# 0xMiden/miden-vm

Measured on AMD Instinct MI355X. Metric: trace rows/sec proved (2^20-row trace, 96-bit sec), higher is better.
Workload: dtype u64 (Goldilocks field, p = 2^64 - 2^32 + 1); 1 GPU; full proof of miden:20:51:8 (DummyMidenAir 2^20 x 51 + 8 EF aux), 96-bit production PCS params (blowup 8, FRI arity 4, 27 queries, PoW 4/12/16), Poseidon2 LMCS; trace resident in HBM, transcript on host; log_trace_rows=20, main_width=51, aux_width_ef=8, log_blowup=3, proof_bytes=137697, parallelism=1 GPU

## Files before the change

### miden-vm_amd/csrc/deep.hip

```cpp
#include "gl.cuh"
#include "kernels.hpp"

__global__ __launch_bounds__(256) void k_bary_weights(const u64* tw, int log_n, u64 g, e2 y0, e2 y1, u64* w0, u64* w1) {
  const size_t n = (size_t)1 << log_n;
  const size_t base = (size_t)blockIdx.x * 1024 + threadIdx.x;
  const size_t half = n >> 1;
  u64 xs[4], nrm[8], pre[8];
  e2 den[8];
#pragma unroll
  for (int k = 0; k < 4; k++) {
    size_t r = base + (size_t)k * 256;
    u64 x = 0;
    if (r < n) x = gl_mul(g, half ? (r < half ? tw[r] : gl_neg(tw[r - half])) : 1);
    xs[k] = x;
    den[2 * k] = e2_sub(y0, e2_make(x));
    den[2 * k + 1] = e2_sub(y1, e2_make(x));
  }
  u64 run = 1;
#pragma unroll
  for (int k = 0; k < 8; k++) {
    nrm[k] = gl_sub(gl_sqr(den[k].c0), gl_mul7(gl_sqr(den[k].c1)));
    pre[k] = run;
    run = gl_mul(run, nrm[k]);
  }
  u64 inv = gl_inv(run);
#pragma unroll
  for (int k = 7; k >= 0; k--) {
    u64 ni = gl_mul(inv, pre[k]);
    inv = gl_mul(inv, nrm[k]);
    size_t r = base + (size_t)(k >> 1) * 256;
    if (r < n) {
      u64 s = gl_mul(ni, xs[k >> 1]);
      u64* w = (k & 1) ? w1 : w0;
      w[2 * r] = gl_mul(den[k].c0, s);
      w[2 * r + 1] = gl_mul(gl_neg(den[k].c1), s);
    }
  }
}

static constexpr int OOD_ROWS_PER_BLOCK = 8192;
__global__ __launch_bounds__(256) void k_ood_partial(const u64* lde, int log_n, int log_blowup, const u64* w0, const u64* w1,
                                                     u64* partial, unsigned chunks) {
  __shared__ u64 red[4][256];
  const size_t n = (size_t)1 << log_n;
  const size_t col = blockIdx.y, chunk = blockIdx.x;
  const u64* f = lde + ((col << log_blowup) << log_n);
  const size_t r0 = chunk * OOD_ROWS_PER_BLOCK;
  const size_t r1 = r0 + OOD_ROWS_PER_BLOCK < n ? r0 + OOD_ROWS_PER_BLOCK : n;
  e2 a0 = e2_make(0), a1 = e2_make(0);
  for (size_t r = r0 + threadIdx.x; r < r1; r += 256) {
    u64 v = f[r];
    a0 = e2_add(a0, e2_mulf(e2{w0[2 * r], w0[2 * r + 1]}, v));
    a1 = e2_add(a1, e2_mulf(e2{w1[2 * r], w1[2 * r + 1]}, v));
  }
  red[0][threadIdx.x] = a0.c0; red[1][threadIdx.x] = a0.c1; red[2][threadIdx.x] = a1.c0; red[3][threadIdx.x] = a1.c1;
  __syncthreads();
  for (int s = 128; s > 0; s >>= 1) {
    if ((int)threadIdx.x < s) {
#pragma unroll
      for (int k = 0; k < 4; k++) red[k][threadIdx.x] = gl_add(red[k][threadIdx.x], red[k][threadIdx.x + s]);
    }
    __syncthreads();
  }
  if (threadIdx.x < 4) partial[(col * chunks + chunk) * 4 + threadIdx.x] = red[threadIdx.x][0];
}

void deep_ood_eval_batch(mh_ctx* c, std::vector<OodJob>& jobs, int log_blowup) {
  struct Weights {
    int log_n;
    size_t coset0;
    e2 y0, y1;
    DevBuf w0, w1;
  };
  std::vector<std::unique_ptr<Weights>> weights;
  struct Slot {
    size_t off = 0, ncol = 0;
    unsigned chunks = 0;
  };
  std::vector<Slot> slots(jobs.size());
  size_t total = 0;
  for (size_t k = 0; k < jobs.size(); k++) {
    OodJob& j = jobs[k];
    const LdeMatrix& m = *j.m;
    if (j.col_end > m.width) j.col_end = m.width;
    j.out0.assign(m.width, e2_make(0));
    j.out1.assign(m.width, e2_make(0));
    if (j.col_begin >= j.col_end) continue;
    const size_t n = (size_t)1 << m.log_n;
    slots[k].ncol = j.col_end - j.col_begin;
    slots[k].chunks = (unsigned)((n + OOD_ROWS_PER_BLOCK - 1) / OOD_ROWS_PER_BLOCK);
    slots[k].off = total;
    total += slots[k].ncol * slots[k].chunks * 4;
  }
  if (!total) return;
  DevBuf partial(total * 8), one;
  for (size_t k = 0; k < jobs.size(); k++) {
    if (!slots[k].ncol) continue;
    const OodJob& j = jobs[k];
    const LdeMatrix& m = *j.m;
    const int log_n = m.log_n;
    const size_t n = (size_t)1 << log_n;
    const u64 g = gl_mul(gl_lde_shift(log_n + log_blowup), gl_pow(gl_two_adic_generator(log_n + log_blowup), m.coset0));
    const u64* tw = log_n ? c->twiddles(log_n, false) : nullptr;
    if (!tw) {
      if (!one.p) {
        one.alloc(8);
        u64 v = 1;
        c->h2d(one.p, &v, 8);
      }
      tw = one.u();
    }
    ProfScope ps(c, "deep_ood_eval", (double)n * 8.0 * slots[k].ncol + 64.0 * n);
    Weights* w = nullptr;
    for (auto& cand : weights)
      if (cand->log_n == log_n && cand->coset0 == m.coset0 && e2_eq(cand->y0, j.y0) && e2_eq(cand->y1, j.y1)) w = cand.get();
    if (!w) {
      weights.emplace_back(new Weights{log_n, m.coset0, j.y0, j.y1, DevBuf(n * 16), DevBuf(n * 16)});
      w = weights.back().get();
      MH_LAUNCH(k_bary_weights, dim3((unsigned)((n + 1023) / 1024)), dim3(256), 0, c->stream, tw, log_n, g, j.y0, j.y1, w->w0.u(), w->w1.u());
    }
    MH_LAUNCH(k_ood_partial, dim3(slots[k].chunks, (unsigned)slots[k].ncol), dim3(256), 0, c->stream,
              m.lde.u() + ((j.col_begin << m.log_cosets) << log_n), log_n, m.log_cosets, w->w0.u(), w->w1.u(), partial.u() + slots[k].off,
              slots[k].chunks);
  }
  std::vector<u64> host(total);
  c->d2h(host.data(), partial.p, total * 8);
  for (size_t k = 0; k < jobs.size(); k++) {
    if (!slots[k].ncol) continue;
    OodJob& j = jobs[k];
    const LdeMatrix& m = *j.m;
    const int log_n = m.log_n;
    const size_t n = (size_t)1 << log_n;
    const u64 g = gl_mul(gl_lde_shift(log_n + log_blowup), gl_pow(gl_two_adic_generator(log_n + log_blowup), m.coset0));
    const u64 g_inv = gl_inv(g), n_inv = gl_inv((u64)n % GL_P);
    const e2 s0 = e2_mulf(e2_sub(e2_exp_pow2(e2_mulf(j.y0, g_inv), log_n), e2_make(1)), n_inv);
    const e2 s1 = e2_mulf(e2_sub(e2_exp_pow2(e2_mulf(j.y1, g_inv), log_n), e2_make(1)), n_inv);
    for (size_t col = 0; col < slots[k].ncol; col++) {
      e2 a0 = e2_make(0), a1 = e2_make(0);
      for (unsigned ch = 0; ch < slots[k].chunks; ch++) {
        const u64* p = host.data() + slots[k].off + (col * slots[k].chunks + ch) * 4;
        a0 = e2_add(a0, e2{p[0], p[1]});
        a1 = e2_add(a1, e2{p[2], p[3]});
      }
      j.out0[j.col_begin + col] = e2_mul(a0, s0);
      j.out1[j.col_begin + col] = e2_mul(a1, s1);
    }
  }
}
void deep_ood_eval_matrix(mh_ctx* c, const LdeMatrix& m, int log_blowup, e2 y0, e2 y1, std::vector<e2>& out0, std::vector<e2>& out1,
                          size_t col_begin, size_t col_end) {
  std::vector<OodJob> jobs(1);
  jobs[0].m = &m; jobs[0].y0 = y0; jobs[0].y1 = y1; jobs[0].col_begin = col_begin; jobs[0].col_end = col_end;
  deep_ood_eval_batch(c, jobs, log_blowup);
  out0.swap(jobs[0].out0);
  out1.swap(jobs[0].out1);
}

static constexpr int DEEP_MAX_MATS = 128;
static constexpr unsigned DEEP_FLUSH = 128;
#ifndef DEEP_UNROLL
#define DEEP_UNROLL 2
#endif
#ifndef DEEP_PTS_N
#define DEEP_PTS_N 1
#endif
static constexpr int DEEP_PTS = DEEP_PTS_N;
struct DeepMat {
  const u64* lde;
  u32 width, coef_off;
  int log_n;
};
struct DeepArgs {
  DeepMat m[DEEP_MAX_MATS];
  int n_mats, log_n, log_blowup;
  const u64* negc;
  const u64* tw;
  const u64* coset_x;
  e2 z0, z1, fred0, fred1, beta;
  u64* out;
};

template <bool PLANES>
__global__ __launch_bounds__(256) void k_deep_assemble(DeepArgs a) {
  const size_t N = (size_t)1 << a.log_n;
  const size_t j = blockIdx.y;
  const size_t base = (size_t)blockIdx.x * (256 * DEEP_PTS) + threadIdx.x;
  size_t r[DEEP_PTS];
#pragma unroll
  for (int k = 0; k < DEEP_PTS; k++) r[k] = base + (size_t)k * 256;
  e2 neg[DEEP_PTS];
  u64 w[DEEP_PTS][2][6];
#pragma unroll
  for (int k = 0; k < DEEP_PTS; k++) {
    neg[k] = e2_make(0);
#pragma unroll
    for (int e = 0; e < 2; e++)
#pragma unroll
      for (int i = 0; i < 6; i++) w[k][e][i] = 0;
  }
  auto flush = [&]() {
    const u64 C[6] = {1ULL, 1ULL << 22, 1ULL << 44, 1ULL << 32, 1ULL << 54, GL_EPS << 12};
#pragma unroll
    for (int k = 0; k < DEEP_PTS; k++) {
      u64 s0 = w[k][0][0], s1 = w[k][1][0];
#pragma unroll
      for (int i = 1; i < 6; i++) {
        s0 = gl_add(s0, gl_mul(w[k][0][i], C[i]));
        s1 = gl_add(s1, gl_mul(w[k][1][i], C[i]));
      }
      neg[k] = e2_add(neg[k], e2{s0, s1});
#pragma unroll
      for (int e = 0; e < 2; e++)
#pragma unroll
        for (int i = 0; i < 6; i++) w[k][e][i] = 0;
    }
  };
  u32 pending = 0;
#pragma unroll 1
  for (int mi = 0; mi < a.n_mats; mi++) {
    const DeepMat m = a.m[mi];
    const size_t nm_mask = ((size_t)1 << m.log_n) - 1;
    const u64* colp = m.lde + (j << m.log_n);
    const size_t cstride = (size_t)1 << (m.log_n + a.log_blowup);
#pragma unroll DEEP_UNROLL
    for (u32 cidx = 0; cidx < m.width; cidx++) {
      const u64 cf0 = a.negc[2 * (m.coef_off + cidx)], cf1 = a.negc[2 * (m.coef_off + cidx) + 1];
      u32 al[2][3];
#pragma unroll
      for (int i = 0; i < 3; i++) {
        al[0][i] = (u32)(cf0 >> (22 * i)) & 0x3FFFFFu;
        al[1][i] = (u32)(cf1 >> (22 * i)) & 0x3FFFFFu;
      }
#pragma unroll
      for (int k = 0; k < DEEP_PTS; k++) {
        if (r[k] < N) {
          const u64 v = colp[r[k] & nm_mask];
          const u32 v0 = (u32)v, v1 = (u32)(v >> 32);
#pragma unroll
          for (int e = 0; e < 2; e++) {
            w[k][e][0] += (u64)al[e][0] * v0;
            w[k][e][1] += (u64)al[e][1] * v0;
            w[k][e][2] += (u64)al[e][2] * v0;
            w[k][e][3] += (u64)al[e][0] * v1;
            w[k][e][4] += (u64)al[e][1] * v1;
            w[k][e][5] += (u64)al[e][2] * v1;
          }
        }
      }
      colp += cstride;
      if (++pending == DEEP_FLUSH) {
        flush();
        pending = 0;
      }
    }
  }
  flush();
  const size_t half = N >> 1;
  const u64 cx = a.coset_x[j];
  e2 den[2 * DEEP_PTS];
  u64 nrm[2 * DEEP_PTS], pre[2 * DEEP_PTS];
#pragma unroll
  for (int k = 0; k < DEEP_PTS; k++) {
    u64 x = 0;
    if (r[k] < N) x = gl_mul(cx, half ? (r[k] < half ? a.tw[r[k]] : gl_neg(a.tw[r[k] - half])) : 1);
    den[2 * k] = e2_sub(a.z0, e2_make(x));
    den[2 * k + 1] = e2_sub(a.z1, e2_make(x));
  }
  u64 run = 1;
#pragma unroll
  for (int k = 0; k < 2 * DEEP_PTS; k++) {
    nrm[k] = gl_sub(gl_sqr(den[k].c0), gl_mul7(gl_sqr(den[k].c1)));
    pre[k] = run;
    run = gl_mul(run, nrm[k]);
  }
  u64 inv = gl_inv(run);
  e2 qinv[2 * DEEP_PTS];
#pragma unroll
  for (int k = 2 * DEEP_PTS - 1; k >= 0; k--) {
    u64 ni = gl_mul(inv, pre[k]);
    inv = gl_mul(inv, nrm[k]);
    qinv[k] = e2{gl_mul(den[k].c0, ni), gl_mul(gl_neg(den[k].c1), ni)};
  }
#pragma unroll
  for (int k = 0; k < DEEP_PTS; k++) {
    if (r[k] < N) {
      e2 v = e2_mul(qinv[2 * k], e2_add(a.fred0, neg[k]));
      v = e2_add(v, e2_mul(e2_mul(a.beta, qinv[2 * k + 1]), e2_add(a.fred1, neg[k])));
      if constexpr (PLANES) {
        a.out[r[k]] = v.c0;
        a.out[N + r[k]] = v.c1;
      } else {
        ulonglong2* o = reinterpret_cast<ulonglong2*>(a.out + 2 * ((j << a.log_n) + r[k]));
        *o = make_ulonglong2(v.c0, v.c1);
      }
    }
  }
}

__global__ __launch_bounds__(256) void k_deep_interleave(const u64* __restrict__ planes, size_t n, u64* __restrict__ out) {
  const size_t i = (size_t)blockIdx.x * 256 + threadIdx.x;
  if (i >= n) return;
  *reinterpret_cast<ulonglong2*>(out + 2 * i) = make_ulonglong2(planes[i], planes[n + i]);
}

void deep_assemble(mh_ctx* c, const std::vector<const LdeMatrix*>& mats, const std::vector<u32>& coef_off, int log_n, int log_blowup,
                   const std::vector<e2>& negc, e2 z0, e2 z1, e2 fred0, e2 fred1, e2 beta, u64* out, bool one_coset) {
  MH_REQUIRE(mats.size() <= (size_t)DEEP_MAX_MATS, "too many committed matrices for one DEEP pass");
  const int lbl = mats[0]->log_cosets;
  const size_t coset0 = mats[0]->coset0;
  for (auto* m : mats) MH_REQUIRE(m->log_cosets == lbl && m->coset0 == coset0, "internal: matrices cover different cosets");
  const size_t N = (size_t)1 << log_n, B = (size_t)1 << lbl;
  const int L = log_n + log_blowup;
  std::vector<u64> blob;
  for (e2 v : negc) { blob.push_back(v.c0); blob.push_back(v.c1); }
  const size_t o_cx = blob.size();
  const u64 g = gl_lde_shift(L), wK = gl_two_adic_generator(L);
  u64 x = gl_mul(g, gl_pow(wK, coset0));
  for (size_t j = 0; j < B; j++) {
    blob.push_back(x);
    x = gl_mul(x, wK);
  }
  DevBuf dblob(blob.size() * 8), one;
  c->h2d(dblob.p, blob.data(), blob.size() * 8);
  const u64* tw = log_n ? c->twiddles(log_n, false) : nullptr;
  if (!tw) {
    one.alloc(8);
    u64 v = 1;
    c->h2d(one.p, &v, 8);
    tw = one.u();
  }
  MH_REQUIRE(!one_coset || (lbl >= 1 && log_n >= DEEP_ONE_COSET_MIN_LOG_N), "internal: one-coset DEEP assemble needs two cosets to extend to");
  const size_t Ba = one_coset ? 1 : B;
  DeepArgs a{};
  double bytes = 16.0 * N * Ba;
  for (size_t i = 0; i < mats.size(); i++) {
    a.m[i] = DeepMat{mats[i]->lde.u(), (u32)mats[i]->width, coef_off[i], mats[i]->log_n};
    bytes += 8.0 * (double)mats[i]->width * (double)(((size_t)1 << mats[i]->log_n) * Ba);
  }
  a.n_mats = (int)mats.size();
  a.log_n = log_n; a.log_blowup = lbl;
  a.negc = dblob.u(); a.tw = tw; a.coset_x = dblob.u() + o_cx;
  a.z0 = z0; a.z1 = z1; a.fred0 = fred0; a.fred1 = fred1; a.beta = beta; a.out = out;
  const dim3 grid((unsigned)((N + 256 * DEEP_PTS - 1) / (256 * DEEP_PTS)), (unsigned)Ba);
  if (!one_coset) {
    ProfScope ps(c, "deep_assemble", bytes);
    MH_LAUNCH(k_deep_assemble<false>, grid, dim3(256), 0, c->stream, a);
    HIP_CHECK(hipStreamSynchronize(c->stream));
    return;
  }
  DevBuf planes(2 * N * 8), scratch(2 * N * 8), ext(2 * B * N * 8);
  a.out = planes.u();
  {
    ProfScope ps(c, "deep_assemble", bytes);
    MH_LAUNCH(k_deep_assemble<true>, grid, dim3(256), 0, c->stream, a);
  }
  {
    ProfScope ps(c, "deep_extend", 16.0 * N + 3.0 * 16.0 * N * B);
    const std::vector<u64> shifts(blob.begin() + o_cx, blob.begin() + o_cx + B);
    lde_columns(c, planes.u(), 2, log_n, shifts[0], shifts, ext.u(), scratch.u());
    MH_LAUNCH(k_deep_interleave, dim3((unsigned)((B * N + 255) / 256)), dim3(256), 0, c->stream, ext.u(), B * N, out);
  }
  HIP_CHECK(hipStreamSynchronize(c->stream));
}
```

Baseline: 24.98 million trace rows/s.

## Group OOD columns per block and use lazy limb-split accumulation

Adds a grouped out-of-domain evaluation kernel in which each block handles several columns at once, so each barycentric weight load is reused across the group. It also drops per-row Goldilocks reductions: each weight is split into 22-bit limbs and multiplied against 32-bit halves of the value, and the products are accumulated in plain 64-bit sums that are reduced only once at the end. A static assertion bounds the accumulators so no mid-loop flush is needed. The grouped path is on by default and can be turned off with an environment variable. The cost is more registers per thread and a tighter occupancy hint.

```diff
diff --git a/miden-vm_amd/csrc/deep.hip b/miden-vm_amd/csrc/deep.hip
--- a/miden-vm_amd/csrc/deep.hip
+++ b/miden-vm_amd/csrc/deep.hip
@@ -63,6 +63,83 @@
     __syncthreads();
   }
   if (threadIdx.x < 4) partial[(col * chunks + chunk) * 4 + threadIdx.x] = red[threadIdx.x][0];
+}
+
+#ifndef OOD_GROUP_N
+#define OOD_GROUP_N 4
+#endif
+static constexpr int OOD_GROUP = OOD_GROUP_N;
+static constexpr int OOD_ROWS_PER_LANE = OOD_ROWS_PER_BLOCK / 256;
+static_assert(OOD_ROWS_PER_BLOCK % 256 == 0 && (u64)OOD_ROWS_PER_LANE * 2 * 0x3FFFFFULL * 0xFFFFFFFFULL < (1ULL << 60),
+              "k_ood_partial_grouped: an accumulator must stay canonical without a flush");
+__device__ __forceinline__ u64 ood_shift32(u64 w) {
+  const u32 a = (u32)w, b = (u32)(w >> 32);
+  const u32 t = a + b, c = t < a;
+  const u32 sub = b + c;
+  return ((u64)(t + c - (sub != 0)) << 32) | (u32)(0u - sub);
+}
+template <int G>
+__global__ __launch_bounds__(256) __attribute__((amdgpu_waves_per_eu(4))) void k_ood_partial_grouped(
+    const u64* lde, int log_n, int log_blowup, const u64* w0, const u64* w1, u64* partial, unsigned chunks, unsigned ncol) {
+  __shared__ u64 red[4][256];
+  const size_t n = (size_t)1 << log_n;
+  const size_t chunk = blockIdx.x;
+  const unsigned col0 = blockIdx.y * G;
+  const u64* f[G];
+#pragma unroll
+  for (int g = 0; g < G; g++) {
+    const size_t col = col0 + g < ncol ? col0 + g : ncol - 1;
+    f[g] = lde + ((col << log_blowup) << log_n);
+  }
+  const size_t r0 = chunk * OOD_ROWS_PER_BLOCK;
+  const size_t r1 = r0 + OOD_ROWS_PER_BLOCK < n ? r0 + OOD_ROWS_PER_BLOCK : n;
+  u64 acc[G][4][3];
+#pragma unroll
+  for (int g = 0; g < G; g++)
+#pragma unroll
+    for (int k = 0; k < 4; k++)
+#pragma unroll
+      for (int i = 0; i < 3; i++) acc[g][k][i] = 0;
+  for (size_t r = r0 + threadIdx.x; r < r1; r += 256) {
+    const ulonglong2 wa = *reinterpret_cast<const ulonglong2*>(w0 + 2 * r), wb = *reinterpret_cast<const ulonglong2*>(w1 + 2 * r);
+    u32 v0[G], v1[G];
+#pragma unroll
+    for (int g = 0; g < G; g++) {
+      const u64 v = f[g][r];
+      v0[g] = (u32)v;
+      v1[g] = (u32)(v >> 32);
+    }
+    const u64 wk[4] = {wa.x, wa.y, wb.x, wb.y};
+#pragma unroll
+    for (int k = 0; k < 4; k++) {
+      const u64 ws = ood_shift32(wk[k]);
+#pragma unroll
+      for (int i = 0; i < 3; i++) {
+        const u32 l = (u32)(wk[k] >> (22 * i)) & 0x3FFFFFu, ls = (u32)(ws >> (22 * i)) & 0x3FFFFFu;
+#pragma unroll
+        for (int g = 0; g < G; g++) {
+          acc[g][k][i] += (u64)l * v0[g];
+          acc[g][k][i] += (u64)ls * v1[g];
+        }
+      }
+    }
+  }
+#pragma unroll
+  for (int g = 0; g < G; g++) {
+    if (g) __syncthreads();
+#pragma unroll
+    for (int k = 0; k < 4; k++)
+      red[k][threadIdx.x] = gl_add(gl_add(acc[g][k][0], gl_mul(acc[g][k][1], 1ULL << 22)), gl_mul(acc[g][k][2], 1ULL << 44));
+    __syncthreads();
+    for (int s = 128; s > 0; s >>= 1) {
+      if ((int)threadIdx.x < s) {
+#pragma unroll
+        for (int k = 0; k < 4; k++) red[k][threadIdx.x] = gl_add(red[k][threadIdx.x], red[k][threadIdx.x + s]);
+      }
+      __syncthreads();
+    }
+    if (threadIdx.x < 4 && col0 + g < ncol) partial[((size_t)(col0 + g) * chunks + chunk) * 4 + threadIdx.x] = red[threadIdx.x][0];
+  }
 }
 
 void deep_ood_eval_batch(mh_ctx* c, std::vector<OodJob>& jobs, int log_blowup) {
@@ -94,6 +171,11 @@
   }
   if (!total) return;
   DevBuf partial(total * 8), one;
+  const char* grouped_env = getenv("MH_OOD_GROUPED");
+  const bool grouped = !(grouped_env && grouped_env[0] && !atoi(grouped_env));
+  if (grouped) {
+    ProfScope mark(c, "ood_grouped");
+  }
   for (size_t k = 0; k < jobs.size(); k++) {
     if (!slots[k].ncol) continue;
     const OodJob& j = jobs[k];
@@ -119,9 +201,14 @@
       w = weights.back().get();
       MH_LAUNCH(k_bary_weights, dim3((unsigned)((n + 1023) / 1024)), dim3(256), 0, c->stream, tw, log_n, g, j.y0, j.y1, w->w0.u(), w->w1.u());
     }
-    MH_LAUNCH(k_ood_partial, dim3(slots[k].chunks, (unsigned)slots[k].ncol), dim3(256), 0, c->stream,
-              m.lde.u() + ((j.col_begin << m.log_cosets) << log_n), log_n, m.log_cosets, w->w0.u(), w->w1.u(), partial.u() + slots[k].off,
-              slots[k].chunks);
+    const u64* lde0 = m.lde.u() + ((j.col_begin << m.log_cosets) << log_n);
+    if (grouped)
+      MH_LAUNCH(k_ood_partial_grouped<OOD_GROUP>, dim3(slots[k].chunks, (unsigned)((slots[k].ncol + OOD_GROUP - 1) / OOD_GROUP)), dim3(256),
+                0, c->stream, lde0, log_n, m.log_cosets, w->w0.u(), w->w1.u(), partial.u() + slots[k].off, slots[k].chunks,
+                (unsigned)slots[k].ncol);
+    else
+      MH_LAUNCH(k_ood_partial, dim3(slots[k].chunks, (unsigned)slots[k].ncol), dim3(256), 0, c->stream, lde0, log_n, m.log_cosets,
+                w->w0.u(), w->w1.u(), partial.u() + slots[k].off, slots[k].chunks);
   }
   std::vector<u64> host(total);
   c->d2h(host.data(), partial.p, total * 8);
```

After: 24.98 million trace rows/s, median of 2. No clear change (-0.0%).
